# PixelClear/OclPathTracer

Measured on AMD Instinct MI355X. Metric: Msamples/sec (pixels x spp / s), cornellbox.bin 1024x1024, higher is better.
Workload: dtype f32; 1 GPU; BASELINE configs[2]: cornellbox.bin 1024x1024, 256 spp, depth 16, full path; render_lanes=2, checkpointed_launches=True, staging_ring_bytes=402653184, workspace_bytes=510711120

## Files before the change

oclpathtracer_amd/csrc/pt_kernels.h:

```cpp
#pragma once

#include <hip/hip_runtime.h>
#include <stddef.h>
#include <stdint.h>

struct PtRawTriangle { float p1[4], p2[4], p3[4]; int32_t id; char pad[12]; };
struct PtRawMaterial { float albedo[4], emissive[4]; float roughness; int32_t type; char pad[24]; };
static_assert(sizeof(PtRawTriangle) == 64 && sizeof(PtRawMaterial) == 64, "record layout");

struct PtPrepTriangle {
    float p1[3];
    float e1[3];
    float e2[3];
    float pad0[3];
    float n[3];
    int32_t id;
};
static_assert(sizeof(PtPrepTriangle) == 64, "prep layout");

struct PtBvhNode {
    float lmin[3]; uint32_t link_l;
    float lmax[3]; uint32_t link_r;
    float rmin[3]; uint32_t pad0;
    float rmax[3]; uint32_t pad1;
// ... 121 lines not shown
    bool det_bounded;
    int quads;
};
hipError_t ptk_trace(const PtTraceParams& p, int num_blocks, PtSearchMode m, bool tally, bool wide, hipStream_t s);
#define PT_BVH_NEAR_EYE 4.0f
hipError_t ptk_bvh_big_raw(const PtRawTriangle* raw, const int* bigidx, int nbig, PtRawTriangle* out, hipStream_t s);
static inline size_t ptk_bvh_record_count(int ntri) { return 2 * (size_t)(ntri > 0 ? ntri : 0); }
size_t ptk_bvh_temp_bytes(int ntri);
#define PT_BVH_BIG_MAX 64
#define PT_BVH_RAY_EPS 1.2e-4f
hipError_t ptk_bvh_build(const PtRawTriangle* raw, const PtPrepTriangle* prep, int ntri, PtBvh8Node* recs,
                         PtPrepTriangle* bigtab, int* bigidx, int* nbig_dev, PtBvhGrid* grid_dev, unsigned* used_dev, void* temp, size_t temp_bytes,
                         hipStream_t s);
#define PT_DET_BOUND_MAX 2.0e19f
#define PT_BVH_AUTO_MIN 512
hipError_t ptk_fold(const PtFoldParams& p, hipStream_t s);
hipError_t ptk_assemble_stripes(const float4* gathered, float4* image, int width, int height, int stripe_rows,
                                int n_ranks, int slab_rows, hipStream_t s);
hipError_t ptk_tonemap_ppm(const float4* fb, int32_t* rgb, size_t npix, hipStream_t s);
hipError_t ptk_fill_i32(int32_t* dst, int32_t value, int n, hipStream_t s);
hipError_t ptk_math(const float* in, float* out, int n, hipStream_t s);
hipError_t ptk_fold_check(unsigned long long* out, int mode, unsigned first, unsigned long long count, hipStream_t s);
hipError_t ptk_shade_check(unsigned long long* out, int mode, unsigned first, unsigned long long count, hipStream_t s);
struct PtQueryParams {
    PtTraceParams t;
    const float4* rays;
    void* out;
    uint32_t nrays;
    int32_t occluded;
};
hipError_t ptk_query(const PtQueryParams& q, int bvh_blocks, PtSearchMode m, bool any, hipStream_t s);
int ptk_query_bvh_blocks_per_cu(void);
struct PtAoParams {
    PtTraceParams t;
    PtLensCamera cam;
    unsigned long long* counts;
    uint32_t npix;
    uint32_t nitems;
    int32_t frame0;
    int32_t K;
    float tlim;
};
#pragma clang diagnostic push
#pragma clang diagnostic ignored "-Winvalid-offsetof"
static_assert(offsetof(PtAoParams, cam) == sizeof(PtTraceParams), "PtAoParams begins { t, cam }");
#pragma clang diagnostic pop
// ... 142 lines not shown
```

oclpathtracer_amd/csrc/pt_kernels.hip:

```cpp
#include "pt_kernels.h"

#include "pt_device_math.h"
#include "pt_secmask.h"

#include <type_traits>
#include <utility>

typedef const __attribute__((address_space(4))) float* pt_const_f32p;

PTK_DEV unsigned pt_lane_id() { return __builtin_amdgcn_mbcnt_hi(~0u, __builtin_amdgcn_mbcnt_lo(~0u, 0u)); }
PTK_DEV unsigned pt_mbcnt(unsigned long long m) { return __builtin_amdgcn_mbcnt_hi((unsigned)(m >> 32), __builtin_amdgcn_mbcnt_lo((unsigned)m, 0u)); }

typedef const __attribute__((address_space(4))) PtTraceParams* pt_kargs_p;
PTK_DEV pt_kargs_p pt_kargs()
{
    pt_kargs_p k = (pt_kargs_p)__builtin_amdgcn_kernarg_segment_ptr();
    asm volatile("" : "+s"(k));
    return k;
}
PTK_DEV f3 pt_anchor()
{
    const pt_kargs_p K = pt_kargs();
    return mk3(K->cam.eye[0], K->cam.eye[1], K->cam.eye[2]);
}
// ... 343 lines not shown
                          float& hv, int& hidx)
{
    float pvx = pt_fma(d.y, r.e2z, -(d.z * r.e2y));
    float pvy = pt_fma(d.z, r.e2x, -(d.x * r.e2z));
    float pvz = pt_fma(d.x, r.e2y, -(d.y * r.e2x));
    float det = pt_fma(r.e1z, pvz, pt_fma(r.e1y, pvy, r.e1x * pvx));
    float inv_det = DET_BOUNDED ? pt_rcp_fast(det) : 1.0f / det;
    float tvx = o.x - r.p1x, tvy = o.y - r.p1y, tvz = o.z - r.p1z;
    float u = pt_fma(tvz, pvz, pt_fma(tvy, pvy, tvx * pvx)) * inv_det;
    bool ok = valid & !(det < 1e-8f) & !(u < 0.0f);
    float qvx = pt_fma(tvy, r.e1z, -(tvz * r.e1y));
    float qvy = pt_fma(tvz, r.e1x, -(tvx * r.e1z));
    float qvz = pt_fma(tvx, r.e1y, -(tvy * r.e1x));
    float v = pt_fma(d.z, qvz, pt_fma(d.y, qvy, d.x * qvx)) * inv_det;
    ok &= !(v < 0.0f) & !(u + v > 1.0f);
    float tt = pt_fma(r.e2z, qvz, pt_fma(r.e2y, qvy, r.e2x * qvx)) * inv_det;
    ok &= (tt > 0.0f) & (tt < tmax);
    tmax = ok ? tt : tmax;
    hu = ok ? u : hu;
    hv = ok ? v : hv;
    hidx = ok ? i : hidx;
}

#ifndef PT_TAIL_LANES
#define PT_TAIL_LANES 32
#endif
#define PT_TAIL_LIST 128u

typedef __attribute__((address_space(3))) unsigned pt_lds_u32;
typedef __attribute__((address_space(3))) unsigned long long pt_lds_u64;
struct PtTail {
    pt_lds_u64* keys;
    pt_lds_u32* list;
    unsigned wr, rd;
    unsigned tile;
    unsigned long long kbest;
    float ku, kv;
};

typedef __attribute__((address_space(3))) unsigned short pt_lds_u16;
template <int LDS_TABLE> PTK_DEV unsigned pt_tail_get(const PtTail& tl, unsigned i)
{
    return LDS_TABLE == 1 ? (unsigned)((pt_lds_u16*)tl.list)[i] : tl.list[i];
}
template <int LDS_TABLE> PTK_DEV void pt_tail_put(const PtTail& tl, unsigned i, unsigned pair)
{
// ... 44 lines not shown
    const f3 pd = mk3(pt_from_lane(a, d.x), pt_from_lane(a, d.y), pt_from_lane(a, d.z));
    const PtTriRec r = pt_fetch_rec<(LDS_TABLE == 1 ? 1 : 0)>(tris, (int)tri);
    float t, u, v;
    const bool ok = pt_tri_candidate<DET_BOUNDED>(r, po, pd, t, u, v) & act;
    if (ok) {
        const unsigned long long key = ((unsigned long long)__float_as_uint(t) << 32) | (unsigned long long)((tri << 6) | lane);
        __hip_atomic_fetch_min(tl.keys + ray, key, __ATOMIC_RELAXED, __HIP_MEMORY_SCOPE_WAVEFRONT);
    }
    __builtin_amdgcn_fence(__ATOMIC_RELEASE, "wavefront");
    __builtin_amdgcn_wave_barrier();
    __builtin_amdgcn_fence(__ATOMIC_ACQUIRE, "wavefront");
    const unsigned long long slot = tl.keys[lane];
    const unsigned from = ((unsigned)slot & 63u) << 2;
    const float pu = pt_from_lane(from, u), pv = pt_from_lane(from, v);
    const bool changed = slot != tl.kbest;
    tl.kbest = slot;
    tl.ku = changed ? pu : tl.ku;
    tl.kv = changed ? pv : tl.kv;
    tl.rd += cnt;
}

template <bool DET_BOUNDED, int LDS_TABLE>
PTK_DEV void pt_pass2_chunk(unsigned m, int base, int n, const PtPrepTriangle* tris, const f3& o, const f3& d, float& tmax, float& hu,
                            float& hv, int& hidx, PtTail& tl, unsigned lane, unsigned& steps)
{
    if (LDS_TABLE == 2 && (unsigned)__popcll(PT_LANES(m != 0u)) > (unsigned)PT_TAIL_LANES) pt_stage_tile(tris, base, n, tl.tile, lane);
    for (pt_lanes more = PT_LANES(m != 0u); (unsigned)__popcll(more) > (unsigned)PT_TAIL_LANES; more = PT_LANES(m != 0u)) {
        ++steps;
        const bool valid = m != 0u;
        unsigned lz;
        asm("v_ffbh_u32_e32 %0, %1" : "=v"(lz) : "v"(m));
        const int i = (LDS_TABLE != 0 || valid) ? base + n - 32 + (int)lz : base;
        m &= ~(0x80000000u >> (lz & 31u));
        const PtTriRec r = LDS_TABLE == 2 ? pt_fetch_rec<2>(tris, n - 32 + (int)lz, tl.tile) : pt_fetch_rec<LDS_TABLE>(tris, i);
        pt_tri_pass2<DET_BOUNDED>(r, i, valid, o, d, tmax, hu, hv, hidx);
    }
    if (PT_TAIL_LANES > 0) {
        for (pt_lanes has = PT_LANES(m != 0u); has != 0ull; has = PT_LANES(m != 0u)) {
            if (m != 0u) {
                unsigned lz;
                asm("v_ffbh_u32_e32 %0, %1" : "=v"(lz) : "v"(m));
                m &= ~(0x80000000u >> (lz & 31u));
                const unsigned tri = (unsigned)(base + n - 32) + lz;
                pt_tail_put<LDS_TABLE>(tl, (tl.wr + pt_mbcnt(has)) & (PT_TAIL_LIST - 1u), (tri << 6) | lane);
            }
            tl.wr += (unsigned)__popcll(has);
            if (tl.wr - tl.rd >= 64u) {
                ++steps;
                pt_tail_round<DET_BOUNDED, LDS_TABLE>(tl, 64u, lane, tris, o, d);
            }
        }
    }
}

template <bool DET_BOUNDED, int LDS_TABLE>
PTK_DEV void pt_pass2_finish(const PtPrepTriangle* tris, const f3& o, const f3& d, float& tmax, float& hu, float& hv, int& hidx,
                             PtTail& tl, unsigned lane, unsigned& steps)
{
    if (PT_TAIL_LANES > 0) {
        if (tl.wr != tl.rd) {
            ++steps;
            pt_tail_round<DET_BOUNDED, LDS_TABLE>(tl, tl.wr - tl.rd, lane, tris, o, d);
        }
        if (tl.wr != 0u) {
            __builtin_amdgcn_fence(__ATOMIC_RELEASE, "wavefront");
            __builtin_amdgcn_wave_barrier();
            __builtin_amdgcn_fence(__ATOMIC_ACQUIRE, "wavefront");
            unsigned long long ones;
            asm volatile("v_mov_b64 %0, -1" : "=v"(ones));
            tl.keys[lane] = ones;
            const unsigned long long key = tl.kbest;
            const float kt = __uint_as_float((unsigned)(key >> 32));
            const int ki = (int)((unsigned)key >> 6);
            const bool better = (key != ~0ull) & ((kt < tmax) | ((kt == tmax) & (ki < hidx)));
            tmax = better ? kt : tmax;
            hu = better ? tl.ku : hu;
            hv = better ? tl.kv : hv;
            hidx = better ? ki : hidx;
        }
    }
}

typedef float pt_f2 __attribute__((ext_vector_type(2)));
PTK_DEV pt_f2 pt_pk_mul_lo(pt_f2 a, pt_f2 s) { pt_f2 r; asm("v_pk_mul_f32 %0, %1, %2 op_sel_hi:[0,1]" : "=v"(r) : "v"(a), "s"(s)); return r; }
PTK_DEV pt_f2 pt_pk_mul_hi(pt_f2 a, pt_f2 s) { pt_f2 r; asm("v_pk_mul_f32 %0, %1, %2 op_sel:[1,0] op_sel_hi:[1,1]" : "=v"(r) : "v"(a), "s"(s)); return r; }
PTK_DEV pt_f2 pt_pk_fma_lo(pt_f2 a, pt_f2 s, pt_f2 c) { pt_f2 r; asm("v_pk_fma_f32 %0, %1, %2, %3 op_sel_hi:[0,1,1]" : "=v"(r) : "v"(a), "s"(s), "v"(c)); return r; }
PTK_DEV pt_f2 pt_pk_fma_hi(pt_f2 a, pt_f2 s, pt_f2 c) { pt_f2 r; asm("v_pk_fma_f32 %0, %1, %2, %3 op_sel:[1,0,0] op_sel_hi:[1,1,1]" : "=v"(r) : "v"(a), "s"(s), "v"(c)); return r; }
PTK_DEV pt_f2 pt_pk_fnma_lo(pt_f2 a, pt_f2 s, pt_f2 c) { pt_f2 r; asm("v_pk_fma_f32 %0, %1, %2, %3 op_sel_hi:[0,1,1] neg_lo:[1,0,0] neg_hi:[1,0,0]" : "=v"(r) : "v"(a), "s"(s), "v"(c)); return r; }
PTK_DEV pt_f2 pt_pk_fnma_hi(pt_f2 a, pt_f2 s, pt_f2 c) { pt_f2 r; asm("v_pk_fma_f32 %0, %1, %2, %3 op_sel:[1,0,0] op_sel_hi:[1,1,1] neg_lo:[1,0,0] neg_hi:[1,0,0]" : "=v"(r) : "v"(a), "s"(s), "v"(c)); return r; }
struct PtRay3 { pt_f2 dxy, dzMx, Myz; };

PTK_DEV void pt_quad3_pass1(pt_const_f32p t, const PtRay3& r, pt_f2& un, pt_f2& T)
{
    typedef const __attribute__((address_space(4))) pt_f2* pt_const_f2p;
    pt_const_f2p s = (pt_const_f2p)t;
    pt_f2 dhi_v;
    { const pt_f2 dhi = s[9]; asm("v_pk_mul_f32 %0, %1, 1.0 op_sel_hi:[1,0]" : "=v"(dhi_v) : "s"(dhi)); }
    T = pt_pk_fma_lo(r.dxy, s[0], dhi_v);
    T = pt_pk_fma_hi(r.dxy, s[1], T);
    T = pt_pk_fma_lo(r.dzMx, s[2], T);
    un = pt_pk_mul_hi(r.dzMx, s[3]);
    un = pt_pk_fma_lo(r.Myz, s[4], un);
    un = pt_pk_fma_hi(r.Myz, s[5], un);
    un = pt_pk_fnma_lo(r.dxy, s[6], un);
    un = pt_pk_fnma_hi(r.dxy, s[7], un);
    un = pt_pk_fnma_lo(r.dzMx, s[8], un);
}

#ifndef PT_STAMPS
#define PT_STAMPS 0
#endif
#if PT_STAMPS
#define PT_STAMP(var) do { __builtin_amdgcn_sched_barrier(0); var = __builtin_amdgcn_s_memtime(); __builtin_amdgcn_s_waitcnt(0xC07F); __builtin_amdgcn_sched_barrier(0); } while (0)
#else
#define PT_STAMP(var) do { } while (0)
#endif

template <bool DET_BOUNDED, int LDS_TABLE, int QUADS, bool UNIT_DIR = false>
PTK_DEV unsigned pt_intersect_two_pass(pt_const_f32p T, const PtPrepTriangle* tris, int ntri, const f3& o, const f3& d,
                                       bool alive, float& tmax, float& hu, float& hv, int& hidx,
                                       float delta1, float ray_radius, pt_const_f32p p1tab, float p1_lo, float p1_hi, const f3& anchor,
                                       PtTail tl, unsigned lane,
                                       unsigned long long* vstat = nullptr, unsigned long long* p1_ticks = nullptr)
{
    tl.wr = tl.rd = 0u;
    tl.kbest = ~0ull;
#if PT_STAMPS
    unsigned long long ta = 0, tb = 0;
#endif
    (void)vstat; (void)p1_ticks; (void)ray_radius; (void)p1tab; (void)p1_lo; (void)p1_hi; (void)anchor;
    unsigned steps = 0;
    bool tame = true;
    PtRay3 r3v;
    if (QUADS == 3 && DET_BOUNDED) {
        const f3 oc = mk3(o.x - anchor.x, o.y - anchor.y, o.z - anchor.z);
        const f3 M = cross3(oc, d);
        r3v.dxy = pt_f2{ d.x, d.y }; r3v.dzMx = pt_f2{ d.z, M.x }; r3v.Myz = pt_f2{ M.y, M.z };
    }
    if (QUADS == 3 && DET_BOUNDED) {
// ... 73 lines not shown
                            const float q1 = __builtin_fabsf((h ? unp.y : unp.x) - unA) / deltaP;
                            const float q3 = __builtin_fabsf(((h ? thp.y : thp.x) - dhi) - detA * 1.000002f) / deltaD;
                            r1 = q1 > r1 ? q1 : r1;
                            r3 = q3 > r3 ? q3 : r3;
                        }
                    }
                }
                atomicMax(&vstat[4], (unsigned long long)__float_as_uint(r1));
                atomicMax(&vstat[5], (unsigned long long)__float_as_uint(r3));
            }
        }
#endif
        if (!alive) m = 0u;
#if PT_STAMPS
        PT_STAMP(tb);
        if (p1_ticks) *p1_ticks += tb - ta;
#endif
        pt_pass2_chunk<DET_BOUNDED, LDS_TABLE>(m, base, n, tris, o, d, tmax, hu, hv, hidx, tl, lane, steps);
    }
    pt_pass2_finish<DET_BOUNDED, LDS_TABLE>(tris, o, d, tmax, hu, hv, hidx, tl, lane, steps);
    return steps;
}

template <bool DET_BOUNDED, int LDS_TABLE>
PTK_DEV unsigned pt_intersect_masked(pt_const_f32p T, const PtPrepTriangle* tris, int ntri, const f3& o, const f3& d, bool alive,
                                      float& tmax, float& hu, float& hv, int& hidx, uint2 pm, PtTail tl, unsigned lane,
                                      unsigned long long* vstat = nullptr)
{
    (void)T; (void)vstat;
    tl.wr = tl.rd = 0u;
    tl.kbest = ~0ull;
    unsigned steps = 0;
    for (int base = 0; base < ntri; base += 32) {
        const int n = ntri - base < 32 ? ntri - base : 32;
        unsigned m = base == 0 ? pm.x : pm.y;
#if PT_VALIDATE_FILTER
        if (alive && vstat) {
            unsigned mx = 0u;
            for (int jj = 0; jj < n; ++jj) {
                const PtTriRec r = pt_load_tri(T, base + jj);
                float pvx = pt_fma(d.y, r.e2z, -(d.z * r.e2y));
                float pvy = pt_fma(d.z, r.e2x, -(d.x * r.e2z));
                float pvz = pt_fma(d.x, r.e2y, -(d.y * r.e2x));
                float det = pt_fma(r.e1z, pvz, pt_fma(r.e1y, pvy, r.e1x * pvx));
                bool keep = !(det < 1e-8f || -det > 1e-8f);
                float inv_det = 1.0f / det;
                float tvx = o.x - r.p1x, tvy = o.y - r.p1y, tvz = o.z - r.p1z;
                float u = pt_fma(tvz, pvz, pt_fma(tvy, pvy, tvx * pvx)) * inv_det;
                keep = keep && !(u < 0.0f || u > 1.0f);
                float qvx = pt_fma(tvy, r.e1z, -(tvz * r.e1y));
                float qvy = pt_fma(tvz, r.e1x, -(tvx * r.e1z));
                float qvz = pt_fma(tvx, r.e1y, -(tvy * r.e1x));
                float v = pt_fma(d.z, qvz, pt_fma(d.y, qvy, d.x * qvx)) * inv_det;
                keep = keep && !(v < 0.0f || u + v > 1.0f);
                float tt = pt_fma(r.e2z, qvz, pt_fma(r.e2y, qvy, r.e2x * qvx)) * inv_det;
                keep = keep && (tt > 0.0f && tt < 1e20f);
                mx |= (keep ? 1u : 0u) << (n - 1 - jj);
            }
            atomicAdd(&vstat[0], (unsigned long long)n);
            atomicAdd(&vstat[1], (unsigned long long)__popc(mx));
            atomicAdd(&vstat[2], (unsigned long long)__popc(m));
            atomicAdd(&vstat[3], (unsigned long long)__popc(mx & ~m));
        }
#endif
        if (!alive) m = 0u;
        pt_pass2_chunk<DET_BOUNDED, LDS_TABLE>(m, base, n, tris, o, d, tmax, hu, hv, hidx, tl, lane, steps);
    }
    pt_pass2_finish<DET_BOUNDED, LDS_TABLE>(tris, o, d, tmax, hu, hv, hidx, tl, lane, steps);
    return steps;
}


struct PtPath {
    f3 o, d;
    f3 mask, L;
    uint32_t seed;
    int bounce;
    unsigned ro;
    unsigned fl;
};

PTK_DEV unsigned pt_ring_offset(unsigned lp, unsigned frame)
{
    const pt_kargs_p KR = pt_kargs();
    const unsigned fr = frame + KR->ring_phase, S = KR->slot_frames;
    const unsigned r = fr - __umulhi(fr, KR->ring_magic) * (2u * S);
    const bool upper = r >= S;
    return (upper ? KR->rad1_off : 0u) + ((upper ? r - S : r) * KR->npix_local + lp) * 12u;
}


// ... 539 lines not shown
    }
    const unsigned wave_in_wg = pt_wave_in_wg();
    constexpr unsigned NW = pt_hit_words<LDS_TABLE>();
    float4* pool = reinterpret_cast<float4*>(pt_lds_tab + pt_lds_pools<LDS_TABLE>(ntri) + wave_in_wg * pt_pool_dwords<LDS_TABLE>());
    unsigned pool_n = 0u;
    PtTail tl = pt_tail_init((pt_lds_u32*)pt_lds_tab + pt_lds_tails<LDS_TABLE>(ntri) + (threadIdx.x >> 6) * pt_lds_tail_dw<LDS_TABLE>(),
                             pt_lds_tiles<LDS_TABLE>(ntri) + (threadIdx.x >> 6) * PT_LDS_TILE_DW, lane);

    PtWaveQueue q = { 0u, 0u, 0u, 0u, 0u, 0u, 0u, 0u };
    pt_lanes alive = 0ull;
    PtPath s = pt_path_idle();
    PtHit h = { 0.0f, 0.0f, -1 };
    pt_lanes ended = 0ull;
    unsigned n_rays = 0, n_samples = 0, n_carried = 0;
    const unsigned wave = pt_wave();
    if (wave < P.carry_in_waves) {
        bool resumed = false;
        pt_carry_hit_load<true, NW>(P, pt_carry_region(P.carry, wave, PT_CARRY_HIT_STRIDE_DW), lane, s, h, resumed, q, n_rays, n_samples, n_carried);
        alive = PT_LANES(resumed);
    }
    q.g = wave & (PT_QUEUE_SHARDS - 1u);
#if PT_STAMPS
    unsigned long long t0 = 0, t1 = 0, t2 = 0, t3 = 0, c_regen = 0, c_loop = 0, c_shade = 0, c_iters = 0, c_steps = 0, c_p1 = 0;
#endif

    for (;;) {
        PT_STAMP(t0);
        {
            const pt_lanes missed = alive & PT_LANES(h.hidx < 0);
            if (PT_ON(missed)) pt_shade_miss(s);
            const pt_lanes over = missed | ended;
            if (PT_ON(over)) pt_path_finish(s);
            n_samples += (unsigned)__popcll(over);
            alive &= ~missed;
            ended = 0ull;
        }
        bool fresh = false;
        bool primary = false;
        unsigned pix0 = 0u;
        if (~alive != 0ull) {
            if (pool_n == 0u && (unsigned)__popcll(alive) <= (unsigned)PT_POOL) {
                const int next = pt_queue_next<true>(P, lane, q, s, alive);
                if (next != 0) {
                    pt_pool_push<NW>(pool, pool_n, s, h, alive);
                    if (next == 2) break;
                    primary = pt_start_fresh<true>(P, lane, q, s, alive, pix0);
// ... 46 lines not shown
                        const uint2 v = *reinterpret_cast<const uint2*>(base + (size_t)(entry * 8u + (unsigned)(PT_SM_HEAD_ENTRIES * 8)));
                        if (covered) pm = v;
#if PT_VALIDATE_FILTER
                        if (P.stats) {
                            const pt_lanes unc = PT_LANES(!covered);
                            if (lane == (unsigned)__builtin_ctzll(alive)) {
                                atomicAdd(&P.stats[10], (unsigned long long)__popcll(alive));
                                atomicAdd(&P.stats[11], (unsigned long long)__popcll(unc & alive));
                            }
                        }
#endif
                    }
                    masked = true;
#if PT_STAMPS
                    PT_STAMP(tb);
                    c_p1 += tb - ta;
#endif
                }
            }
        }
        if (alive == 0ull) {
        } else if (masked)
            p2steps = pt_intersect_masked<DET_BOUNDED, LDS_TABLE>(T, P.tris, ntri, s.o, s.d, PT_ON(alive), tmax, hu, hv, hidx, pm, tl, lane,
                                                                  PT_VALIDATE_FILTER && P.stats ? P.stats + 2 : nullptr);
        else
            p2steps = pt_intersect_two_pass<DET_BOUNDED, LDS_TABLE, QUADS, PT_TRACE_UNIT_DIR != 0>(T, P.tris, ntri, s.o, s.d, PT_ON(alive), tmax, hu, hv, hidx,
                                                                                          P.quad_delta1, P.ray_radius,
                                                                                          (pt_const_f32p)P.p1tab, P.p1_lo, P.p1_hi, pt_anchor(), tl, lane,
                                                                                          PT_VALIDATE_FILTER && P.stats ? P.stats + 2 : nullptr,
#if PT_STAMPS
                                                                                          &c_p1
#else
                                                                                          nullptr
#endif
                                                                                          );
#if PT_STAMPS
        c_steps += p2steps;
#else
        (void)p2steps;
#endif

        s.o = add3(s.o, scale3(s.d, tmax));
        h.hu = hu; h.hv = hv; h.hidx = hidx;
#if PT_STAMPS
        PT_STAMP(t3);
        c_regen += t1 - t0; c_shade += t2 - t1; c_loop += t3 - t2; c_iters++;
#endif
    }

#if PT_STAMPS
    if (P.stats && lane == 0) {
        atomicAdd(&P.stats[2], c_regen);
        atomicAdd(&P.stats[3], c_loop);
        atomicAdd(&P.stats[4], c_shade);
        atomicAdd(&P.stats[5], c_iters);
        atomicAdd(&P.stats[7], c_steps);
        atomicAdd(&P.stats[6], c_p1);
    }
#endif
    {
        const pt_kargs_p K = pt_kargs();
        if (K->carry_out != 0u) {
            pt_carry_store<NW>(pt_carry_region(K->carry, wave, PT_CARRY_HIT_STRIDE_DW), lane, pool, pool_n, q, n_rays, n_samples, n_carried);
            return;
        }
    }
#if !PT_STAMPS && !PT_VALIDATE_FILTER
    if (P.stats && lane == 0 && n_carried != 0u) atomicAdd(&P.stats[7], (unsigned long long)n_carried);
#endif
    pt_flush_counters(P, lane, n_rays, n_samples);
}

#ifndef PT_TRACE_WAVES
#define PT_TRACE_WAVES 8
#endif
template <bool DET_BOUNDED, int LDS_TABLE, int QUADS>
__global__ __launch_bounds__(PT_TRACE_THREADS) __attribute__((amdgpu_waves_per_eu(PT_TRACE_WAVES, PT_TRACE_WAVES)))
void pt_trace_kernel(const PtTraceParams P)
{
    pt_trace_body<DET_BOUNDED, LDS_TABLE, QUADS>(P);
// ... 706 lines not shown
            const float b2 = __uint_as_float((eb2 << 23) | mb2);
            if (k == 4u) a = 0.0f;
            const bool a_in = pt_div_in_window(__float_as_uint(a)), b_in = pt_div_in_window(__float_as_uint(b));
            ++seen;
            inside += a_in && b_in;
            differ(pt_div(a, b), a / b, a);
            if (a_in || k == 4u) differ(pt_div_by(a, b), a / b, a);
            const float a0 = a * c;
            float q0, q1;
            pt_div_pair(a0, b, a, b2, q0, q1);
            differ(q0, a0 / b, a);
            differ(q1, a / b2, a);
        }
    }
    if (bad) {
        atomicAdd(out + (mode == 1 ? 1 : mode == 3 ? 3 : 2), (unsigned long long)bad);
        atomicMax(out + 6, (unsigned long long)worst_hi);
        atomicMax(out + 7, (unsigned long long)worst_lo);
    }
    if (seen) atomicAdd(out + 4, (unsigned long long)seen);
    if (inside) atomicAdd(out + 5, (unsigned long long)inside);
}

__global__ void pt_assemble_kernel(const float4* __restrict__ gathered, float4* __restrict__ image, int width,
                                   int height, int stripe_rows, int n_ranks, int slab_rows)
{
    size_t i = (size_t)blockIdx.x * blockDim.x + threadIdx.x;
    size_t total = (size_t)width * height;
    if (i >= total) return;
    unsigned row = (unsigned)(i / (unsigned)width);
    unsigned x = (unsigned)(i - (size_t)row * width);
    unsigned stripe = row / (unsigned)stripe_rows;
    unsigned within = row - stripe * (unsigned)stripe_rows;
    unsigned rank = stripe % (unsigned)n_ranks;
    unsigned sl = stripe / (unsigned)n_ranks;
    size_t src = ((size_t)rank * slab_rows + (size_t)sl * stripe_rows + within) * width + x;
    image[i] = gathered[src];
}

PTK_DEV int32_t pt_f2c(float v)
{
    float a = __builtin_sqrtf(v) * 255.0f;
    int32_t i;
    if (a != a) i = (int32_t)0x80000000;
    else if (a >= 2147483648.0f) i = (int32_t)0x80000000;
    else if (a <= -2147483648.0f) i = (int32_t)0x80000000;
// ... 1930 lines not shown
hipError_t ptk_tonemap_ppm(const float4* fb, int32_t* rgb, size_t npix, hipStream_t s)
{
    if (npix == 0) return hipSuccess;
    hipLaunchKernelGGL(pt_tonemap_kernel, dim3((unsigned)((npix + 255) / 256)), dim3(256), 0, s, fb, rgb, npix);
    return hipGetLastError();
}

hipError_t ptk_fold_check(unsigned long long* out, int mode, unsigned first, unsigned long long count, hipStream_t s)
{
    if (count == 0) return hipSuccess;
    const unsigned long long want = (count + 255) / 256;
    hipLaunchKernelGGL(pt_fold_check_kernel, dim3((unsigned)(want < 65536ull ? want : 65536ull)), dim3(256), 0, s, out, mode, first, count);
    return hipGetLastError();
}

hipError_t ptk_shade_check(unsigned long long* out, int mode, unsigned first, unsigned long long count, hipStream_t s)
{
    if (count == 0) return hipSuccess;
    const unsigned long long want = (count + 255) / 256;
    hipLaunchKernelGGL(pt_shade_check_kernel, dim3((unsigned)(want < 65536ull ? want : 65536ull)), dim3(256), 0, s, out, mode, first, count);
    return hipGetLastError();
}

hipError_t ptk_math(const float* in, float* out, int n, hipStream_t s)
{
    if (n <= 0) return hipSuccess;
    hipLaunchKernelGGL(pt_math_kernel, dim3((n + 255) / 256), dim3(256), 0, s, in, out, n);
    return hipGetLastError();
}

hipError_t ptk_fill_i32(int32_t* dst, int32_t value, int n, hipStream_t s)
{
    if (n <= 0) return hipSuccess;
    hipLaunchKernelGGL(pt_fill_i32_kernel, dim3((n + 255) / 256), dim3(256), 0, s, dst, value, n);
    return hipGetLastError();
}

size_t ptk_trace_lds_bytes(int ntri)
{
    return (size_t)(ntri <= PT_LDS_TRI_MAX ? pt_lds_total<1>(ntri) : pt_lds_total<2>(ntri)) * sizeof(float);
}

size_t ptk_trace_bvh_lds_bytes(void)
{
    return (size_t)pt_bvh_lds_total() * sizeof(float);
}
// ... 216 lines not shown
```

oclpathtracer_amd/csrc/pt_shim.hip:

```cpp
#include "../../include/pt_shim.h"

#include <hip/hip_runtime.h>

#include <algorithm>
#include <cmath>
#include <cstdarg>
#include <cstdio>
#include <cstdlib>
#include <cstring>
#include <initializer_list>
#include <new>
#include <string>
#include <utility>
#include <vector>

#include "pt_denoise.h"
#include "pt_reproject.h"
#include "pt_kernels.h"
#include "pt_secmask.h"

static thread_local char g_err[512] = "";

static int fail(int code, const char* fmt, ...)
{
    va_list ap;
    va_start(ap, fmt);
    vsnprintf(g_err, sizeof g_err, fmt, ap);
    va_end(ap);
    return code;
}

#define HIP_TRY(expr)                                                                          \
    do {                                                                                       \
        hipError_t e_ = (expr);                                                                \
        if (e_ != hipSuccess) return fail(PT_ERR_HIP, "%s failed: %s", #expr, hipGetErrorString(e_)); \
    } while (0)

extern "C" const char* pt_last_error(void) { return g_err; }
extern "C" int pt_abi_version(void) { return PT_SHIM_ABI_VERSION; }

enum { KERNEL_GENERATE_COLORS = 0, KERNEL_FILL = 1, KERNEL_MATH = 2, KERNEL_FOLD_CHECK = 3, KERNEL_SHADE_CHECK = 4, KERNEL_COUNT = 5 };

struct pt_kernel_s {
    int id;
    const char* file;
    const char* func;
};

struct pt_buffer_s {
    pt_device_s* dev;
    void* dptr;
    size_t bytes;
    bool owned;
    uint64_t version;
    void* staging;
    size_t staging_bytes;
    bool mapped;
    size_t mapped_bytes;
    bool exposed;
};

struct pt_event_s {
    pt_device_s* dev;
    hipEvent_t start, stop;
// ... 224 lines not shown
        snprintf(arch, sizeof arch, "%s", d->prop.gcnArchName);
        delete d;
        return fail(PT_ERR_NO_DEVICE, "device %d is %s; this library carries gfx950 (MI355X) code only", device_idx, arch);
    }
    if (hipStreamCreateWithFlags(&d->own_stream, hipStreamNonBlocking) != hipSuccess) {
        delete d;
        return fail(PT_ERR_HIP, "hipStreamCreate failed");
    }
    d->stream = d->own_stream;
    d->opt_batch = 1;
    d->opt_pmask = PT_DEFAULT_PRIMARY_MASKS;
    d->opt_smask = PT_DEFAULT_SECONDARY_MASKS;
    d->opt_denoise = PT_DENOISE_GATHER_AUTO;
    d->opt_denoise_spatial = PT_DENOISE_POOL_AUTO;
    d->opt_reproject = PT_REPROJECT_FORM_AUTO;
    d->opt_bvh_stack = 64;
    d->opt_lanes = 2;
    d->opt_carry = 1;
    d->kernels[KERNEL_GENERATE_COLORS] = { KERNEL_GENERATE_COLORS, "GenerateColors", "GenerateColors" };
    d->kernels[KERNEL_FILL] = { KERNEL_FILL, "PtShimTest", "FillKernel" };
    d->kernels[KERNEL_MATH] = { KERNEL_MATH, "PtShimTest", "MathKernel" };
    d->kernels[KERNEL_FOLD_CHECK] = { KERNEL_FOLD_CHECK, "PtShimTest", "FoldCheckKernel" };
    d->kernels[KERNEL_SHADE_CHECK] = { KERNEL_SHADE_CHECK, "PtShimTest", "ShadeCheckKernel" };
    bool ok = ws_malloc(d, d->bigtab, WS_BIGTAB) == hipSuccess && ws_malloc(d, d->bigidx, WS_BIGIDX) == hipSuccess &&
              ws_malloc(d, d->counters, WS_COUNTERS) == hipSuccess && ws_malloc(d, d->big_filter.p1tab, ws_big_p1tab()) == hipSuccess &&
              ws_malloc(d, d->det_bound_dev, WS_DETBOUND) == hipSuccess;
    for (int k = 0; ok && k < 2; ++k)
        ok = hipStreamCreateWithFlags(&d->lane[k], hipStreamNonBlocking) == hipSuccess &&
             hipEventCreateWithFlags(&d->ev_fold[k], hipEventDisableTiming) == hipSuccess &&
             hipEventCreateWithFlags(&d->ev_slot[k], hipEventDisableTiming) == hipSuccess;
    ok = ok && hipEventCreateWithFlags(&d->ev_fork, hipEventDisableTiming) == hipSuccess &&
         hipEventCreateWithFlags(&d->ev_ext, hipEventDisableTiming) == hipSuccess;
    ok = ok && hipHostMalloc(reinterpret_cast<void**>(&d->trav_host), 64, hipHostMallocMapped) == hipSuccess &&
         hipHostGetDevicePointer(reinterpret_cast<void**>(&d->trav_dev), d->trav_host, 0) == hipSuccess;
    if (ok) {
        d->trav_host[0] = d->trav_host[1] = 0u;
        ok = hipMemsetAsync(d->counters, 0, WS_COUNTERS, d->own_stream) == hipSuccess && hipStreamSynchronize(d->own_stream) == hipSuccess;
    }
    if (!ok) {
        (void)hipGetLastError();
        destroy_device_objects(d);
        return fail(PT_ERR_OOM, "workspace allocation failed");
    }
    d->blocks_per_cu = ptk_trace_blocks_per_cu(36);
    d->bvh_blocks_per_cu = ptk_trace_bvh_blocks_per_cu();
    d->query_bvh_blocks_per_cu = ptk_query_bvh_blocks_per_cu();
// ... 2431 lines not shown
}

static int launch_shade_check(pt_device_s* d, const pt_launch_arg* a, int nargs, pt_event_s* ev)
{
    if (nargs != 4 || !a[0].is_buffer || a[1].is_buffer || a[1].size != 4 || a[2].is_buffer || a[2].size != 4 || a[3].is_buffer ||
        a[3].size != 8)
        return fail(PT_ERR_ARGS, "ShadeCheckKernel expects (buffer, int, uint, ulong)");
    pt_buffer_s* out = a[0].buffer;
    if (!out || out->dev != d || out->bytes < 8 * sizeof(unsigned long long)) return fail(PT_ERR_ARGS, "ShadeCheckKernel: bad buffer");
    int32_t mode;
    uint32_t first;
    uint64_t count;
    memcpy(&mode, a[1].data, 4);
    memcpy(&first, a[2].data, 4);
    memcpy(&count, a[3].data, 8);
    if (mode < 1 || mode > 3) return fail(PT_ERR_ARGS, "ShadeCheckKernel: mode %d", mode);
    int rc = enter_stream(d);
    if (rc || (rc = event_begin(d, ev))) return rc;
    HIP_TRY(ptk_shade_check((unsigned long long*)out->dptr, mode, first, count, d->stream));
    out->version++;
    return event_end(d, ev);
}

extern "C" int pt_launch_2d(pt_device_t d, pt_kernel_t k, const pt_launch_arg* args, int nargs, int ntx, int nty, int lx,
                            int ly, pt_event_t ev, float* ms_out)
{
    int rc = use_device(d);
    if (rc) return rc;
    if (!k) return fail(PT_ERR_NOT_FOUND, "null kernel (Device::getKernel returned 0)");
    if (k < d->kernels || k >= d->kernels + KERNEL_COUNT) return fail(PT_ERR_INVALID, "kernel belongs to another device");
    if (nargs < 0 || nargs > PT_MAX_ARG_COUNT || (nargs && !args)) return fail(PT_ERR_ARGS, "bad argument list");
    for (int i = 0; i < nargs; ++i)
        if (!args[i].is_buffer && args[i].size > PT_MAX_ARG_SIZE) return fail(PT_ERR_ARGS, "constant %d larger than %d bytes", i, PT_MAX_ARG_SIZE);
    if (ntx < 0 || nty < 0 || lx < 1 || ly < 1) return fail(PT_ERR_ARGS, "bad launch geometry");
    if (ev && ev->dev != d) return fail(PT_ERR_INVALID, "event belongs to another device");
    long long n = (long long)ntx * nty;
    if (ms_out) *ms_out = 0.f;
    switch (k->id) {
    case KERNEL_GENERATE_COLORS: return launch_generate_colors(d, args, nargs, n, ev, ms_out);
    case KERNEL_FILL: return launch_fill(d, args, nargs, n, ev);
    case KERNEL_MATH: return launch_math(d, args, nargs, n, ev);
    case KERNEL_FOLD_CHECK: return launch_fold_check(d, args, nargs, ev);
    case KERNEL_SHADE_CHECK: return launch_shade_check(d, args, nargs, ev);
    default: return fail(PT_ERR_NOT_FOUND, "unknown kernel id");
    }
}
```

Measured before the change: 10740 Msamples/s.

## Build masked-intersection tail list by pairing lanes across both mask words

For the LDS-table masked intersection path, the per-32-triangle chunk loop is replaced by a single own-lane pass with a lower tail threshold. It is followed by a paired list builder that compacts rays with remaining candidates and lets two lanes split each ray's low and high mask words via ds_permute/bpermute. This aims to cut the serial iterations spent appending candidate (triangle, ray) pairs to the tail ring, giving better lane utilization when few rays carry many candidates. It also adds a PairCheck test kernel and finer stamp instrumentation, and costs extra permute instructions and register pressure.

```diff
diff --git a/oclpathtracer_amd/csrc/pt_kernels.h b/oclpathtracer_amd/csrc/pt_kernels.h
--- a/oclpathtracer_amd/csrc/pt_kernels.h
+++ b/oclpathtracer_amd/csrc/pt_kernels.h
@@ -167,6 +167,7 @@
 hipError_t ptk_math(const float* in, float* out, int n, hipStream_t s);
 hipError_t ptk_fold_check(unsigned long long* out, int mode, unsigned first, unsigned long long count, hipStream_t s);
 hipError_t ptk_shade_check(unsigned long long* out, int mode, unsigned first, unsigned long long count, hipStream_t s);
+hipError_t ptk_pair_check(const uint2* masks, unsigned* out, int ntri, unsigned cases, unsigned cap, hipStream_t s);
 struct PtQueryParams {
     PtTraceParams t;
     const float4* rays;
diff --git a/oclpathtracer_amd/csrc/pt_kernels.hip b/oclpathtracer_amd/csrc/pt_kernels.hip
--- a/oclpathtracer_amd/csrc/pt_kernels.hip
+++ b/oclpathtracer_amd/csrc/pt_kernels.hip
@@ -389,6 +389,16 @@
     hidx = ok ? i : hidx;
 }
 
+#ifndef PT_STAMPS
+#define PT_STAMPS 0
+#endif
+#if PT_STAMPS
+#define PT_STAMP(var) do { __builtin_amdgcn_sched_barrier(0); var = __builtin_amdgcn_s_memtime(); __builtin_amdgcn_s_waitcnt(0xC07F); __builtin_amdgcn_sched_barrier(0); } while (0)
+#else
+#define PT_STAMP(var) do { } while (0)
+#endif
+struct PtStampSplit { unsigned long long own, append, rounds, finish, iters, searches; };
+
 #ifndef PT_TAIL_LANES
 #define PT_TAIL_LANES 32
 #endif
@@ -479,8 +489,13 @@
 
 template <bool DET_BOUNDED, int LDS_TABLE>
 PTK_DEV void pt_pass2_chunk(unsigned m, int base, int n, const PtPrepTriangle* tris, const f3& o, const f3& d, float& tmax, float& hu,
-                            float& hv, int& hidx, PtTail& tl, unsigned lane, unsigned& steps)
-{
+                            float& hv, int& hidx, PtTail& tl, unsigned lane, unsigned& steps, PtStampSplit* sp = nullptr)
+{
+    (void)sp;
+#if PT_STAMPS
+    unsigned long long s0 = 0, s1 = 0, s2 = 0, ra = 0, rb = 0, rsum = 0;
+    PT_STAMP(s0);
+#endif
     if (LDS_TABLE == 2 && (unsigned)__popcll(PT_LANES(m != 0u)) > (unsigned)PT_TAIL_LANES) pt_stage_tile(tris, base, n, tl.tile, lane);
     for (pt_lanes more = PT_LANES(m != 0u); (unsigned)__popcll(more) > (unsigned)PT_TAIL_LANES; more = PT_LANES(m != 0u)) {
         ++steps;
@@ -492,8 +507,12 @@
         const PtTriRec r = LDS_TABLE == 2 ? pt_fetch_rec<2>(tris, n - 32 + (int)lz, tl.tile) : pt_fetch_rec<LDS_TABLE>(tris, i);
         pt_tri_pass2<DET_BOUNDED>(r, i, valid, o, d, tmax, hu, hv, hidx);
     }
+    PT_STAMP(s1);
     if (PT_TAIL_LANES > 0) {
         for (pt_lanes has = PT_LANES(m != 0u); has != 0ull; has = PT_LANES(m != 0u)) {
+#if PT_STAMPS
+            if (sp) sp->iters++;
+#endif
             if (m != 0u) {
                 unsigned lz;
                 asm("v_ffbh_u32_e32 %0, %1" : "=v"(lz) : "v"(m));
@@ -504,21 +523,36 @@
             tl.wr += (unsigned)__popcll(has);
             if (tl.wr - tl.rd >= 64u) {
                 ++steps;
+                PT_STAMP(ra);
                 pt_tail_round<DET_BOUNDED, LDS_TABLE>(tl, 64u, lane, tris, o, d);
+#if PT_STAMPS
+                PT_STAMP(rb);
+                rsum += rb - ra;
+#endif
             }
         }
     }
+#if PT_STAMPS
+    PT_STAMP(s2);
+    if (sp) { sp->own += s1 - s0; sp->append += (s2 - s1) - rsum; sp->rounds += rsum; }
+#endif
 }
 
 template <bool DET_BOUNDED, int LDS_TABLE>
 PTK_DEV void pt_pass2_finish(const PtPrepTriangle* tris, const f3& o, const f3& d, float& tmax, float& hu, float& hv, int& hidx,
-                             PtTail& tl, unsigned lane, unsigned& steps)
-{
+                             PtTail& tl, unsigned lane, unsigned& steps, PtStampSplit* sp = nullptr)
+{
+    (void)sp;
+#if PT_STAMPS
+    unsigned long long s0 = 0, s1 = 0, s2 = 0;
+    PT_STAMP(s0);
+#endif
     if (PT_TAIL_LANES > 0) {
         if (tl.wr != tl.rd) {
             ++steps;
             pt_tail_round<DET_BOUNDED, LDS_TABLE>(tl, tl.wr - tl.rd, lane, tris, o, d);
         }
+        PT_STAMP(s1);
         if (tl.wr != 0u) {
             __builtin_amdgcn_fence(__ATOMIC_RELEASE, "wavefront");
             __builtin_amdgcn_wave_barrier();
@@ -536,6 +570,10 @@
             hidx = better ? ki : hidx;
         }
     }
+#if PT_STAMPS
+    PT_STAMP(s2);
+    if (sp) { sp->rounds += s1 - s0; sp->finish += s2 - s1; }
+#endif
 }
 
 typedef float pt_f2 __attribute__((ext_vector_type(2)));
@@ -563,15 +601,6 @@
     un = pt_pk_fnma_hi(r.dxy, s[7], un);
     un = pt_pk_fnma_lo(r.dzMx, s[8], un);
 }
-
-#ifndef PT_STAMPS
-#define PT_STAMPS 0
-#endif
-#if PT_STAMPS
-#define PT_STAMP(var) do { __builtin_amdgcn_sched_barrier(0); var = __builtin_amdgcn_s_memtime(); __builtin_amdgcn_s_waitcnt(0xC07F); __builtin_amdgcn_sched_barrier(0); } while (0)
-#else
-#define PT_STAMP(var) do { } while (0)
-#endif
 
 template <bool DET_BOUNDED, int LDS_TABLE, int QUADS, bool UNIT_DIR = false>
 PTK_DEV unsigned pt_intersect_two_pass(pt_const_f32p T, const PtPrepTriangle* tris, int ntri, const f3& o, const f3& d,
@@ -691,51 +720,165 @@
     return steps;
 }
 
+#ifndef PT_PAIR_LIST
+#define PT_PAIR_LIST 2
+#endif
+#ifndef PT_PAIR_TAIL_LANES
+#define PT_PAIR_TAIL_LANES (PT_TAIL_LANES < 24 ? PT_TAIL_LANES : 24)
+#endif
+template <int LDS_TABLE, class ROUND>
+PTK_DEV unsigned pt_pair_list_build(unsigned lo, unsigned hi, int ntri, PtTail& tl, unsigned lane, ROUND&& round)
+{
+    const bool mine = (lo | hi) != 0u;
+    const pt_lanes owners = PT_LANES(mine);
+    if (owners == 0ull) return 0u;
+    const int off_lo = (ntri < 32 ? ntri : 32) - 32, off_hi = ntri - 32;
+    unsigned iters = 0u;
+    if (PT_PAIR_LIST < 2) {
+        for (pt_lanes has = owners; has != 0ull; has = PT_LANES((lo | hi) != 0u)) {
+            ++iters;
+            if ((lo | hi) != 0u) {
+                const bool low = lo != 0u;
+                unsigned m = low ? lo : hi, lz;
+                asm("v_ffbh_u32_e32 %0, %1" : "=v"(lz) : "v"(m));
+                m &= ~(0x80000000u >> (lz & 31u));
+                lo = low ? m : lo;
+                hi = low ? hi : m;
+                pt_tail_put<LDS_TABLE>(tl, (tl.wr + pt_mbcnt(has)) & (PT_TAIL_LIST - 1u), ((unsigned)((low ? off_lo : off_hi) + (int)lz) << 6) | lane);
+            }
+            tl.wr += (unsigned)__popcll(has);
+            if (tl.wr - tl.rd >= 64u) round(64u);
+        }
+        return iters;
+    }
+    const unsigned n_owners = (unsigned)__popcll(owners);
+    const unsigned rank = pt_mbcnt(owners);
+    const unsigned dest = mine ? rank : n_owners + lane - rank;
+    const unsigned owner_at = (unsigned)__builtin_amdgcn_ds_permute((int)(dest << 2), (int)lane);
+    const unsigned own_bits = (lane & 1u) ? 0x55555555u : 0xAAAAAAAAu;
+    const unsigned pair_lo = (unsigned)off_lo << 6, pair_hi = (unsigned)(off_hi - off_lo) << 6;
+    for (unsigned first = 0u; first < n_owners; first += 32u) {
+        const unsigned k = first + (lane >> 1);
+        const unsigned ray = (unsigned)__builtin_amdgcn_ds_bpermute((int)(k << 2), (int)owner_at);
+        const unsigned wlo = (unsigned)__builtin_amdgcn_ds_bpermute((int)(ray << 2), (int)lo);
+        const unsigned whi = (unsigned)__builtin_amdgcn_ds_bpermute((int)(ray << 2), (int)hi);
+        unsigned m = k < n_owners ? (wlo & own_bits) | (whi & ~own_bits) : 0u;
+        for (pt_lanes has = PT_LANES(m != 0u); has != 0ull; has = PT_LANES(m != 0u)) {
+            ++iters;
+            if (m != 0u) {
+                unsigned lz;
+                asm("v_ffbh_u32_e32 %0, %1" : "=v"(lz) : "v"(m));
+                m &= ~(0x80000000u >> (lz & 31u));
+                const unsigned high = (lz ^ lane) & 1u;
+                unsigned pair;
+                asm("v_mad_u32_u24 %0, %1, %2, %3" : "=v"(pair) : "v"(high), "s"(pair_hi), "v"((lz << 6) | ray));
+                pair += pair_lo;
+                pt_tail_put<LDS_TABLE>(tl, (tl.wr + pt_mbcnt(has)) & (PT_TAIL_LIST - 1u), pair);
+            }
+            tl.wr += (unsigned)__popcll(has);
+            if (tl.wr - tl.rd >= 64u) round(64u);
+        }
+    }
+    return iters;
+}
+
+#if PT_VALIDATE_FILTER
+PTK_DEV void pt_validate_mask_word(pt_const_f32p T, int base, int n, unsigned m, const f3& o, const f3& d, bool alive, unsigned long long* vstat)
+{
+    if (alive && vstat) {
+        unsigned mx = 0u;
+        for (int jj = 0; jj < n; ++jj) {
+            const PtTriRec r = pt_load_tri(T, base + jj);
+            float pvx = pt_fma(d.y, r.e2z, -(d.z * r.e2y));
+            float pvy = pt_fma(d.z, r.e2x, -(d.x * r.e2z));
+            float pvz = pt_fma(d.x, r.e2y, -(d.y * r.e2x));
+            float det = pt_fma(r.e1z, pvz, pt_fma(r.e1y, pvy, r.e1x * pvx));
+            bool keep = !(det < 1e-8f || -det > 1e-8f);
+            float inv_det = 1.0f / det;
+            float tvx = o.x - r.p1x, tvy = o.y - r.p1y, tvz = o.z - r.p1z;
+            float u = pt_fma(tvz, pvz, pt_fma(tvy, pvy, tvx * pvx)) * inv_det;
+            keep = keep && !(u < 0.0f || u > 1.0f);
+            float qvx = pt_fma(tvy, r.e1z, -(tvz * r.e1y));
+            float qvy = pt_fma(tvz, r.e1x, -(tvx * r.e1z));
+            float qvz = pt_fma(tvx, r.e1y, -(tvy * r.e1x));
+            float v = pt_fma(d.z, qvz, pt_fma(d.y, qvy, d.x * qvx)) * inv_det;
+            keep = keep && !(v < 0.0f || u + v > 1.0f);
+            float tt = pt_fma(r.e2z, qvz, pt_fma(r.e2y, qvy, r.e2x * qvx)) * inv_det;
+            keep = keep && (tt > 0.0f && tt < 1e20f);
+            mx |= (keep ? 1u : 0u) << (n - 1 - jj);
+        }
+        atomicAdd(&vstat[0], (unsigned long long)n);
+        atomicAdd(&vstat[1], (unsigned long long)__popc(mx));
+        atomicAdd(&vstat[2], (unsigned long long)__popc(m));
+        atomicAdd(&vstat[3], (unsigned long long)__popc(mx & ~m));
+    }
+}
+#endif
+
 template <bool DET_BOUNDED, int LDS_TABLE>
 PTK_DEV unsigned pt_intersect_masked(pt_const_f32p T, const PtPrepTriangle* tris, int ntri, const f3& o, const f3& d, bool alive,
                                       float& tmax, float& hu, float& hv, int& hidx, uint2 pm, PtTail tl, unsigned lane,
-                                      unsigned long long* vstat = nullptr)
-{
-    (void)T; (void)vstat;
+                                      unsigned long long* vstat = nullptr, PtStampSplit* sp = nullptr)
+{
+    (void)T; (void)vstat; (void)sp;
     tl.wr = tl.rd = 0u;
     tl.kbest = ~0ull;
     unsigned steps = 0;
-    for (int base = 0; base < ntri; base += 32) {
-        const int n = ntri - base < 32 ? ntri - base : 32;
-        unsigned m = base == 0 ? pm.x : pm.y;
+#if PT_STAMPS
+    if (sp) sp->searches++;
+#endif
+    if (LDS_TABLE == 1 && PT_PAIR_LIST > 0 && PT_PAIR_TAIL_LANES > 0) {
+        const int n = ntri < 32 ? ntri : 32;
+        unsigned m = pm.x, mh = ntri > 32 ? pm.y : 0u;
 #if PT_VALIDATE_FILTER
-        if (alive && vstat) {
-            unsigned mx = 0u;
-            for (int jj = 0; jj < n; ++jj) {
-                const PtTriRec r = pt_load_tri(T, base + jj);
-                float pvx = pt_fma(d.y, r.e2z, -(d.z * r.e2y));
-                float pvy = pt_fma(d.z, r.e2x, -(d.x * r.e2z));
-                float pvz = pt_fma(d.x, r.e2y, -(d.y * r.e2x));
-                float det = pt_fma(r.e1z, pvz, pt_fma(r.e1y, pvy, r.e1x * pvx));
-                bool keep = !(det < 1e-8f || -det > 1e-8f);
-                float inv_det = 1.0f / det;
-                float tvx = o.x - r.p1x, tvy = o.y - r.p1y, tvz = o.z - r.p1z;
-                float u = pt_fma(tvz, pvz, pt_fma(tvy, pvy, tvx * pvx)) * inv_det;
-                keep = keep && !(u < 0.0f || u > 1.0f);
-                float qvx = pt_fma(tvy, r.e1z, -(tvz * r.e1y));
-                float qvy = pt_fma(tvz, r.e1x, -(tvx * r.e1z));
-                float qvz = pt_fma(tvx, r.e1y, -(tvy * r.e1x));
-                float v = pt_fma(d.z, qvz, pt_fma(d.y, qvy, d.x * qvx)) * inv_det;
-                keep = keep && !(v < 0.0f || u + v > 1.0f);
-                float tt = pt_fma(r.e2z, qvz, pt_fma(r.e2y, qvy, r.e2x * qvx)) * inv_det;
-                keep = keep && (tt > 0.0f && tt < 1e20f);
-                mx |= (keep ? 1u : 0u) << (n - 1 - jj);
-            }
-            atomicAdd(&vstat[0], (unsigned long long)n);
-            atomicAdd(&vstat[1], (unsigned long long)__popc(mx));
-            atomicAdd(&vstat[2], (unsigned long long)__popc(m));
-            atomicAdd(&vstat[3], (unsigned long long)__popc(mx & ~m));
-        }
-#endif
-        if (!alive) m = 0u;
-        pt_pass2_chunk<DET_BOUNDED, LDS_TABLE>(m, base, n, tris, o, d, tmax, hu, hv, hidx, tl, lane, steps);
-    }
-    pt_pass2_finish<DET_BOUNDED, LDS_TABLE>(tris, o, d, tmax, hu, hv, hidx, tl, lane, steps);
+        pt_validate_mask_word(T, 0, n, m, o, d, alive, vstat);
+        if (ntri > 32) pt_validate_mask_word(T, 32, ntri - 32, mh, o, d, alive, vstat);
+#endif
+        if (!alive) m = mh = 0u;
+#if PT_STAMPS
+        unsigned long long s0 = 0, s1 = 0, s2 = 0, rsum = 0;
+        PT_STAMP(s0);
+#endif
+        for (pt_lanes more = PT_LANES(m != 0u); (unsigned)__popcll(more) > (unsigned)PT_PAIR_TAIL_LANES; more = PT_LANES(m != 0u)) {
+            ++steps;
+            const bool valid = m != 0u;
+            unsigned lz;
+            asm("v_ffbh_u32_e32 %0, %1" : "=v"(lz) : "v"(m));
+            const int i = n - 32 + (int)lz;
+            m &= ~(0x80000000u >> (lz & 31u));
+            const PtTriRec r = pt_fetch_rec<1>(tris, i);
+            pt_tri_pass2<DET_BOUNDED>(r, i, valid, o, d, tmax, hu, hv, hidx);
+        }
+        PT_STAMP(s1);
+        const unsigned iters = pt_pair_list_build<LDS_TABLE>(m, mh, ntri, tl, lane, [&](unsigned cnt) {
+#if PT_STAMPS
+            unsigned long long ra = 0, rb = 0;
+            PT_STAMP(ra);
+#endif
+            ++steps;
+            pt_tail_round<DET_BOUNDED, LDS_TABLE>(tl, cnt, lane, tris, o, d);
+#if PT_STAMPS
+            PT_STAMP(rb);
+            rsum += rb - ra;
+#endif
+        });
+        (void)iters;
+#if PT_STAMPS
+        PT_STAMP(s2);
+        if (sp) { sp->own += s1 - s0; sp->append += (s2 - s1) - rsum; sp->rounds += rsum; sp->iters += iters; }
+#endif
+    } else {
+        for (int base = 0; base < ntri; base += 32) {
+            const int n = ntri - base < 32 ? ntri - base : 32;
+            unsigned m = base == 0 ? pm.x : pm.y;
+#if PT_VALIDATE_FILTER
+            pt_validate_mask_word(T, base, n, m, o, d, alive, vstat);
+#endif
+            if (!alive) m = 0u;
+            pt_pass2_chunk<DET_BOUNDED, LDS_TABLE>(m, base, n, tris, o, d, tmax, hu, hv, hidx, tl, lane, steps, sp);
+        }
+    }
+    pt_pass2_finish<DET_BOUNDED, LDS_TABLE>(tris, o, d, tmax, hu, hv, hidx, tl, lane, steps, sp);
     return steps;
 }
 
@@ -1321,6 +1464,7 @@
     q.g = wave & (PT_QUEUE_SHARDS - 1u);
 #if PT_STAMPS
     unsigned long long t0 = 0, t1 = 0, t2 = 0, t3 = 0, c_regen = 0, c_loop = 0, c_shade = 0, c_iters = 0, c_steps = 0, c_p1 = 0;
+    PtStampSplit c_split = { 0, 0, 0, 0, 0, 0 };
 #endif
 
     for (;;) {
@@ -1413,7 +1557,13 @@
         if (alive == 0ull) {
         } else if (masked)
             p2steps = pt_intersect_masked<DET_BOUNDED, LDS_TABLE>(T, P.tris, ntri, s.o, s.d, PT_ON(alive), tmax, hu, hv, hidx, pm, tl, lane,
-                                                                  PT_VALIDATE_FILTER && P.stats ? P.stats + 2 : nullptr);
+                                                                  PT_VALIDATE_FILTER && P.stats ? P.stats + 2 : nullptr,
+#if PT_STAMPS
+                                                                  &c_split
+#else
+                                                                  nullptr
+#endif
+                                                                  );
         else
             p2steps = pt_intersect_two_pass<DET_BOUNDED, LDS_TABLE, QUADS, PT_TRACE_UNIT_DIR != 0>(T, P.tris, ntri, s.o, s.d, PT_ON(alive), tmax, hu, hv, hidx,
                                                                                           P.quad_delta1, P.ray_radius,
@@ -1447,6 +1597,12 @@
         atomicAdd(&P.stats[5], c_iters);
         atomicAdd(&P.stats[7], c_steps);
         atomicAdd(&P.stats[6], c_p1);
+        atomicAdd(&P.stats[8], c_split.own);
+        atomicAdd(&P.stats[9], c_split.append);
+        atomicAdd(&P.stats[10], c_split.rounds);
+        atomicAdd(&P.stats[11], c_split.finish);
+        atomicAdd(&P.stats[12], c_split.iters);
+        atomicAdd(&P.stats[13], c_split.searches);
     }
 #endif
     {
@@ -2199,6 +2355,33 @@
     if (inside) atomicAdd(out + 5, (unsigned long long)inside);
 }
 
+__global__ __launch_bounds__(64) void pt_pair_check_kernel(const uint2* __restrict__ masks, unsigned* __restrict__ out, int ntri, unsigned cap)
+{
+    __shared__ __attribute__((aligned(4))) unsigned short ring[PT_TAIL_LIST];
+    const unsigned lane = pt_lane_id();
+    PtTail tl;
+    tl.keys = nullptr;
+    tl.list = (pt_lds_u32*)ring;
+    tl.wr = tl.rd = 0u;
+    tl.kbest = ~0ull; tl.ku = tl.kv = 0.0f;
+    tl.tile = 0u;
+    const uint2 pm = masks[(size_t)blockIdx.x * 64u + lane];
+    unsigned* const o = out + (size_t)blockIdx.x * (2u + cap);
+    unsigned n_out = 0u, rounds = 0u;
+    auto round = [&](unsigned cnt) {
+        __builtin_amdgcn_fence(__ATOMIC_RELEASE, "wavefront");
+        __builtin_amdgcn_wave_barrier();
+        __builtin_amdgcn_fence(__ATOMIC_ACQUIRE, "wavefront");
+        if (lane < cnt && n_out + lane < cap) o[2u + n_out + lane] = pt_tail_get<1>(tl, (tl.rd + lane) & (PT_TAIL_LIST - 1u));
+        n_out += cnt;
+        tl.rd += cnt;
+        ++rounds;
+    };
+    pt_pair_list_build<1>(pm.x, ntri > 32 ? pm.y : 0u, ntri, tl, lane, round);
+    if (tl.wr != tl.rd) round(tl.wr - tl.rd);
+    if (lane == 0u) { o[0] = n_out; o[1] = rounds; }
+}
+
 __global__ void pt_assemble_kernel(const float4* __restrict__ gathered, float4* __restrict__ image, int width,
                                    int height, int stripe_rows, int n_ranks, int slab_rows)
 {
@@ -4175,6 +4358,13 @@
     return hipGetLastError();
 }
 
+hipError_t ptk_pair_check(const uint2* masks, unsigned* out, int ntri, unsigned cases, unsigned cap, hipStream_t s)
+{
+    if (cases == 0) return hipSuccess;
+    hipLaunchKernelGGL(pt_pair_check_kernel, dim3(cases), dim3(64), 0, s, masks, out, ntri, cap);
+    return hipGetLastError();
+}
+
 hipError_t ptk_math(const float* in, float* out, int n, hipStream_t s)
 {
     if (n <= 0) return hipSuccess;
diff --git a/oclpathtracer_amd/csrc/pt_shim.hip b/oclpathtracer_amd/csrc/pt_shim.hip
--- a/oclpathtracer_amd/csrc/pt_shim.hip
+++ b/oclpathtracer_amd/csrc/pt_shim.hip
@@ -39,7 +39,7 @@
 extern "C" const char* pt_last_error(void) { return g_err; }
 extern "C" int pt_abi_version(void) { return PT_SHIM_ABI_VERSION; }
 
-enum { KERNEL_GENERATE_COLORS = 0, KERNEL_FILL = 1, KERNEL_MATH = 2, KERNEL_FOLD_CHECK = 3, KERNEL_SHADE_CHECK = 4, KERNEL_COUNT = 5 };
+enum { KERNEL_GENERATE_COLORS = 0, KERNEL_FILL = 1, KERNEL_MATH = 2, KERNEL_FOLD_CHECK = 3, KERNEL_SHADE_CHECK = 4, KERNEL_PAIR_CHECK = 5, KERNEL_COUNT = 6 };
 
 struct pt_kernel_s {
     int id;
@@ -310,6 +310,7 @@
     d->kernels[KERNEL_MATH] = { KERNEL_MATH, "PtShimTest", "MathKernel" };
     d->kernels[KERNEL_FOLD_CHECK] = { KERNEL_FOLD_CHECK, "PtShimTest", "FoldCheckKernel" };
     d->kernels[KERNEL_SHADE_CHECK] = { KERNEL_SHADE_CHECK, "PtShimTest", "ShadeCheckKernel" };
+    d->kernels[KERNEL_PAIR_CHECK] = { KERNEL_PAIR_CHECK, "PtShimTest", "PairCheckKernel" };
     bool ok = ws_malloc(d, d->bigtab, WS_BIGTAB) == hipSuccess && ws_malloc(d, d->bigidx, WS_BIGIDX) == hipSuccess &&
               ws_malloc(d, d->counters, WS_COUNTERS) == hipSuccess && ws_malloc(d, d->big_filter.p1tab, ws_big_p1tab()) == hipSuccess &&
               ws_malloc(d, d->det_bound_dev, WS_DETBOUND) == hipSuccess;
@@ -2787,6 +2788,29 @@
     return event_end(d, ev);
 }
 
+static int launch_pair_check(pt_device_s* d, const pt_launch_arg* a, int nargs, pt_event_s* ev)
+{
+    if (nargs != 5 || !a[0].is_buffer || !a[1].is_buffer || a[2].is_buffer || a[2].size != 4 || a[3].is_buffer || a[3].size != 4 ||
+        a[4].is_buffer || a[4].size != 4)
+        return fail(PT_ERR_ARGS, "PairCheckKernel expects (buffer, buffer, int, uint, uint)");
+    pt_buffer_s *masks = a[0].buffer, *out = a[1].buffer;
+    if (!masks || !out || masks->dev != d || out->dev != d) return fail(PT_ERR_ARGS, "PairCheckKernel: bad buffer");
+    int32_t ntri;
+    uint32_t cases, cap;
+    memcpy(&ntri, a[2].data, 4);
+    memcpy(&cases, a[3].data, 4);
+    memcpy(&cap, a[4].data, 4);
+    if (ntri < 1 || ntri > 64) return fail(PT_ERR_ARGS, "PairCheckKernel: %d triangles", ntri);
+    if (cases > 65536u || cap > 4096u) return fail(PT_ERR_ARGS, "PairCheckKernel: %u cases of %u pairs", cases, cap);
+    if (masks->bytes < (size_t)cases * 64u * 8u || out->bytes < (size_t)cases * (2u + cap) * 4u)
+        return fail(PT_ERR_ARGS, "PairCheckKernel: buffer too small");
+    int rc = enter_stream(d);
+    if (rc || (rc = event_begin(d, ev))) return rc;
+    HIP_TRY(ptk_pair_check((const uint2*)masks->dptr, (unsigned*)out->dptr, ntri, cases, cap, d->stream));
+    out->version++;
+    return event_end(d, ev);
+}
+
 extern "C" int pt_launch_2d(pt_device_t d, pt_kernel_t k, const pt_launch_arg* args, int nargs, int ntx, int nty, int lx,
                             int ly, pt_event_t ev, float* ms_out)
 {
@@ -2807,6 +2831,7 @@
     case KERNEL_MATH: return launch_math(d, args, nargs, n, ev);
     case KERNEL_FOLD_CHECK: return launch_fold_check(d, args, nargs, ev);
     case KERNEL_SHADE_CHECK: return launch_shade_check(d, args, nargs, ev);
+    case KERNEL_PAIR_CHECK: return launch_pair_check(d, args, nargs, ev);
     default: return fail(PT_ERR_NOT_FOUND, "unknown kernel id");
     }
 }
```

Result: faster. 11170 Msamples/s (median of 6 runs) (+4.0%).
